# david-jk/BigGAN-Tensorflow

Hardware: AMD Instinct MI355X
Metric: BigGAN-128 train-step images/sec (higher is better)
Workload: dtype bf16; 1 GPU; BigGAN-128 ch=96 bf16 (BASELINE config 3: global batch 256, 32/GPU over 8 GPUs); img_size=128, ch=96, per_gpu_batch=256, global_batch=256, da_policy=full, g_regularization=ortho_cosine, n_labels=0, gan_type=hinge, hip_graph=False, precision=bf16, parallelism=dp1

## Files before the change

biggan-tensorflow_amd/csrc/igemm16.hip:

```cpp
#include <stdlib.h>

#include "common.h"
#include "igemm.h"
#include "igemm16.h"
#include <type_traits>
#include "igemm_dev.h"

namespace bg {

typedef float f32x4_t __attribute__((ext_vector_type(4)));
typedef float f32x16_t __attribute__((ext_vector_type(16)));
typedef __bf16 bf16x8_t __attribute__((ext_vector_type(8)));
typedef short s16x4v __attribute__((ext_vector_type(4)));
typedef short s16x8v __attribute__((ext_vector_type(8)));
typedef __attribute__((address_space(3))) void lds_void_t;
typedef __attribute__((address_space(1))) const void gbl_void_t;
typedef __attribute__((address_space(3))) s16x4v lds_s16x4v;

__device__ uint4 g_zero_page[1024];

__device__ __forceinline__ void glds16(const void* src, unsigned char* lds_wave_base) {
    __builtin_amdgcn_global_load_lds((gbl_void_t*)src, (lds_void_t*)lds_wave_base, 16, 0, 0);
}

// ... 1069 lines not shown
    return 256 * row + 16 * (chunk ^ (((row & 3) << 2) | ((row >> 2) & 3)));
}

template <int MODE>
__global__ __launch_bounds__(256, 2) void tn16_kernel(const TN16Params p) {
    constexpr int BM = 128, BN = 128;
    extern __shared__ __attribute__((aligned(16))) unsigned char smem[];

    const int t = threadIdx.x;
    const int lane = t & 63, w = t >> 6;
    const int wm = w >> 1, wn = w & 1;
    const Gather& g = p.g;

    const int ntile = p.tiles_m * p.tiles_n;
    const int lin = xcd_remap(blockIdx.x, ntile * p.splitk);
    const int zs = lin / ntile;
    const int tile = lin - zs * ntile;
    const int tile_n = tile % p.tiles_n, tile_m = tile / p.tiles_n;
    const int mf0 = tile_m * BM, cb0 = tile_n * BN;
    const int row_begin = zs * p.rows_per_split;
    const int row_end = min(p.M, row_begin + p.rows_per_split);
    const int nsteps = max(0, (row_end - row_begin + TN16_BK - 1) / TN16_BK);

    const int prow = lane >> 4;
    const int ch = (lane & 15) ^ ((prow << 2) | w);
    const int mf = mf0 + 8 * ch;
    int a_kh = 0, a_kw = 0, a_c = mf;
    if (MODE != GATHER_PLAIN) {
        const int tap = mf / p.Ca;
        a_c = mf - tap * p.Ca;
        a_kh = tap / g.k;
        a_kw = tap - a_kh * g.k;
    }
    const bool a_ok = mf < p.Mf;
    const int cb = cb0 + 8 * ch;
    const bool b_ok = cb < p.Cb;
    const __bf16* Ab = reinterpret_cast<const __bf16*>(p.A);
    const __bf16* Bb = reinterpret_cast<const __bf16*>(p.Bv);
    const void* zero = reinterpret_cast<const void*>(g_zero_page);
    int m_next = row_begin + 4 * w + prow;

    auto stage = [&](int buf) {
        unsigned char* sa = smem + buf * (2 * TN16_TILE) + (4 * w) * 256;
        unsigned char* sb = sa + TN16_TILE;
#pragma unroll
        for (int j = 0; j < 4; ++j) {
            const int m = m_next + 16 * j;
            const void* srca = zero;
            const void* srcb = zero;
            if (m < row_end) {
                if (a_ok) {
                    int64_t pix;
                    if (MODE == GATHER_PLAIN) {
                        pix = m;
                    } else {
                        int b, ho, wo;
                        if (p.pow2) {
                            wo = m & (g.Wq - 1);
                            const int r = m >> p.wq_shift;
                            ho = r & (g.Hq - 1);
                            b = r >> p.hq_shift;
                        } else {
                            wo = m % g.Wq;
                            const int r = m / g.Wq;
                            ho = r % g.Hq;
                            b = r / g.Hq;
                        }
                        const int hs = conv_src(ho, a_kh, g.stride, g.pad, g.reflect, g.Hs);
                        const int ws = conv_src(wo, a_kw, g.stride, g.pad, g.reflect, g.Ws);
                        pix = (hs >= 0 && ws >= 0) ? ((int64_t)b * g.Hs + hs) * g.Ws + ws : -1;
                    }
                    if (pix >= 0) srca = Ab + pix * g.ld + a_c;
                }
                if (b_ok) srcb = Bb + (int64_t)m * p.b_ld + cb;
            }
            glds16(srca, sa + j * 16 * 256);
            glds16(srcb, sb + j * 16 * 256);
        }
        m_next += TN16_BK;
    };

    f32x16_t acc[2][2];
#pragma unroll
    for (int i = 0; i < 2; ++i)
#pragma unroll
        for (int j = 0; j < 2; ++j)
#pragma unroll
            for (int r = 0; r < 16; ++r) acc[i][j][r] = 0.f;

    const int kblk = lane >> 5, g16 = (lane >> 4) & 1, q = (lane & 15) >> 2, pq = lane & 3;
    const uint32_t lds0 = static_cast<uint32_t>(
        reinterpret_cast<uintptr_t>((__attribute__((address_space(3))) unsigned char*)smem));
    uint32_t a_ad[2][2], b_ad[2][2];
#pragma unroll
    for (int jj = 0; jj < 2; ++jj) {
        const int row = 8 * kblk + 4 * jj + q;
#pragma unroll
        for (int i = 0; i < 2; ++i) {
            a_ad[i][jj] = lds0 + tr16_swz(row, 4 * (wm * 2 + i) + 2 * g16 + (pq >> 1)) + 8 * (pq & 1);
            b_ad[i][jj] = lds0 + TN16_TILE + tr16_swz(row, 4 * (wn * 2 + i) + 2 * g16 + (pq >> 1)) + 8 * (pq & 1);
        }
    }
    auto operand = [&](uint32_t lo_addr, uint32_t hi_addr) {
        const s16x4v lo = lds_tr16(lo_addr), hi = lds_tr16(hi_addr);
        const s16x8v v = __builtin_shufflevector(lo, hi, 0, 1, 2, 3, 4, 5, 6, 7);
        return __builtin_bit_cast(bf16x8_t, v);
    };

    if (nsteps > 0) stage(0);
    __syncthreads();
    for (int it = 0; it < nsteps; ++it) {
        const int cur = it & 1;
        if (it + 1 < nsteps) stage(cur ^ 1);
        const uint32_t bufoff = (uint32_t)cur * (2u * TN16_TILE);
#pragma unroll
        for (int s = 0; s < TN16_BK / 16; ++s) {
            bf16x8_t a[2], b[2];
#pragma unroll
            for (int i = 0; i < 2; ++i) a[i] = operand(a_ad[i][0] + bufoff + 4096 * s, a_ad[i][1] + bufoff + 4096 * s);
#pragma unroll
            for (int j = 0; j < 2; ++j) b[j] = operand(b_ad[j][0] + bufoff + 4096 * s, b_ad[j][1] + bufoff + 4096 * s);
#pragma unroll
            for (int i = 0; i < 2; ++i)
#pragma unroll
                for (int j = 0; j < 2; ++j)
                    acc[i][j] = __builtin_amdgcn_mfma_f32_32x32x16_bf16(a[i], b[j], acc[i][j], 0, 0, 0);
        }
        __syncthreads();
    }

    float* obase = p.out + (int64_t)zs * p.slab_stride;
#pragma unroll
    for (int i = 0; i < 2; ++i) {
#pragma unroll
        for (int r = 0; r < 16; ++r) {
            const int row = mf0 + wm * 64 + 32 * i + (r & 3) + 8 * (r >> 2) + 4 * (lane >> 5);
            if (row >= p.Mf) continue;
#pragma unroll
            for (int j = 0; j < 2; ++j) {
                const int col = cb0 + wn * 64 + 32 * j + (lane & 31);
                if (col < p.Cb) obase[(int64_t)row * p.out_ld + col] = acc[i][j][r];
            }
        }
    }
}


template <int MODE, int BK, int NBI = 1>
__global__ __launch_bounds__(512, (BK == 32 && NBI == 1) ? 4 : 2) void tn16x_kernel(const TN16Params p) {
    constexpr int TILE = BK * 256;
    constexpr int TNX_STAGE = (2 + NBI) * TILE;
    constexpr int NJ = BK / 16;
    extern __shared__ __attribute__((aligned(16))) unsigned char smem[];

    const int t = threadIdx.x;
    const int lane = t & 63, w = t >> 6;
    const int wm = w >> 1, wn = w & 1;
    const Gather& g = p.g;

    const int ntile = p.tiles_m * p.tiles_n;
    const int lin = xcd_remap(blockIdx.x, ntile * p.splitk);
    const int zs = lin / ntile;
    const int tile = lin - zs * ntile;
    const int tile_n = tile % p.tiles_n, tile_m = tile / p.tiles_n;
    const int mf0 = tile_m * 256, cb0 = tile_n * 128 * NBI;
    const int row_begin = zs * p.rows_per_split;
    const int row_end = min(p.M, row_begin + p.rows_per_split);
    const int nsteps = max(0, (row_end - row_begin + BK - 1) / BK);

    const int prow = lane >> 4;
    const int wq = w & 3, ia = w >> 2;
    const int ch = (lane & 15) ^ ((prow << 2) | wq);
    const int mf = mf0 + 128 * ia + 8 * ch;
    int a_kh = 0, a_kw = 0, a_c = mf;
    if (MODE != GATHER_PLAIN) {
        const int tap = mf / p.Ca;
        a_c = mf - tap * p.Ca;
        a_kh = tap / g.k;
        a_kw = tap - a_kh * g.k;
    }
    const int cb = cb0 + (NBI == 2 ? 128 * ia : 0) + 8 * ch;
    const void* zero = reinterpret_cast<const void*>(g_zero_page);
    int m_next = row_begin + 4 * wq + prow;
    const uint32_t lds0 = static_cast<uint32_t>(
        reinterpret_cast<uintptr_t>((__attribute__((address_space(3))) unsigned char*)smem));

    const int dh = a_kh - g.pad, dw = a_kw - g.pad;
    const unsigned hmax = g.reflect ? 0xffffffffu : (unsigned)g.Hs - 1u;
    const unsigned wmax = g.reflect ? 0xffffffffu : (unsigned)g.Ws - 1u;
    const int h2 = 2 * (g.Hs - 1), w2 = 2 * (g.Ws - 1);
    const int wmask = g.Wq - 1, hmask = g.Hq - 1, bsh = p.wq_shift + p.hq_shift;
    const int a_lim = mf < p.Mf ? row_end : 0, b_lim = cb < p.Cb ? row_end : 0;
    const unsigned char* abase = reinterpret_cast<const unsigned char*>(reinterpret_cast<const __bf16*>(p.A) + a_c);
    const unsigned char* bbase = reinterpret_cast<const unsigned char*>(reinterpret_cast<const __bf16*>(p.Bv) + cb);
    const unsigned ald2 = 2u * (unsigned)g.ld, bld2 = 2u * (unsigned)p.b_ld;

    const uint32_t sa0 = __builtin_amdgcn_readfirstlane(lds0 + ia * TILE + (4 * wq) * 256);
    const uint32_t sb0 = __builtin_amdgcn_readfirstlane(lds0 + (2 + (NBI == 2 ? ia : 0)) * TILE + (4 * wq) * 256);
    auto stage = [&](int slot) {
        const uint32_t sa = sa0 + slot * TNX_STAGE;
        const uint32_t sb = sb0 + slot * TNX_STAGE;
#pragma unroll
        for (int j = 0; j < NJ; ++j) {
            const int m = m_next + 16 * j;
            unsigned pix = (unsigned)m;
            bool ok = m < a_lim;
            if (MODE != GATHER_PLAIN) {
                const int wo = m & wmask, ho = (m >> p.wq_shift) & hmask, b = m >> bsh;
                const int h = __mul24(ho, g.stride) + dh, wsrc = __mul24(wo, g.stride) + dw;
                const int ha = h < 0 ? -h : h, wa = wsrc < 0 ? -wsrc : wsrc;
                const int hr = min(ha, h2 - ha), wr = min(wa, w2 - wa);
                ok = ok & ((unsigned)h <= hmax) & ((unsigned)wsrc <= wmax);
                pix = __umul24(__umul24((unsigned)b, (unsigned)g.Hs) + (unsigned)hr, (unsigned)g.Ws) + (unsigned)wr;
            }
            const void* srca = ok ? static_cast<const void*>(abase + (uint64_t)pix * ald2) : zero;
            glds16_asm(srca, sa + j * 16 * 256);
            if (NBI == 2 || j / (NJ / 2) == ia) {
                const void* srcb = m < b_lim ? static_cast<const void*>(bbase + (uint64_t)(unsigned)m * bld2) : zero;
                glds16_asm(srcb, sb + j * 16 * 256);
            }
        }
        m_next += BK;
    };

    constexpr int NBJ = 2 * NBI;
    f32x16_t acc[2][NBJ];
#pragma unroll
    for (int i = 0; i < 2; ++i)
#pragma unroll
        for (int j = 0; j < NBJ; ++j)
#pragma unroll
            for (int r = 0; r < 16; ++r) acc[i][j][r] = 0.f;

    const int kblk = lane >> 5, g16 = (lane >> 4) & 1, q = (lane & 15) >> 2, pq = lane & 3;
    uint32_t a_ad[2][2], b_ad[NBJ][2];
#pragma unroll
    for (int jj = 0; jj < 2; ++jj) {
        const int row = 8 * kblk + 4 * jj + q;
#pragma unroll
        for (int i = 0; i < 2; ++i)
            a_ad[i][jj] = lds0 + (wm >> 1) * TILE +
                          tr16_swz(row, 4 * ((wm & 1) * 2 + i) + 2 * g16 + (pq >> 1)) + 8 * (pq & 1);
#pragma unroll
        for (int j = 0; j < NBJ; ++j)
            b_ad[j][jj] = lds0 + (2 + (NBI == 2 ? wn : 0)) * TILE +
                          tr16_swz(row, 4 * (NBI == 2 ? j : wn * 2 + j) + 2 * g16 + (pq >> 1)) + 8 * (pq & 1);
    }
    auto operand = [&](uint32_t lo_addr, uint32_t hi_addr) {
        const s16x4v lo = lds_tr16(lo_addr), hi = lds_tr16(hi_addr);
        const s16x8v v = __builtin_shufflevector(lo, hi, 0, 1, 2, 3, 4, 5, 6, 7);
        return __builtin_bit_cast(bf16x8_t, v);
    };

    if (nsteps > 0) stage(0);
    if (nsteps > 1) stage(1);
    auto kstep = [&](int it, auto slot_c) {
        constexpr int SLOT = decltype(slot_c)::value;
        if (it + 1 < nsteps) {
            if (BK == 64 && NBI == 2) asm volatile("s_waitcnt vmcnt(8) lgkmcnt(0)" ::: "memory");
            else if (BK == 64) asm volatile("s_waitcnt vmcnt(6) lgkmcnt(0)" ::: "memory");
            else if (NBI == 2) asm volatile("s_waitcnt vmcnt(4) lgkmcnt(0)" ::: "memory");
            else asm volatile("s_waitcnt vmcnt(3) lgkmcnt(0)" ::: "memory");
        } else
            asm volatile("s_waitcnt vmcnt(0) lgkmcnt(0)" ::: "memory");
        __builtin_amdgcn_s_barrier();
        if (it + 2 < nsteps) stage((SLOT + 2) % 3);
        constexpr uint32_t bufoff = (uint32_t)SLOT * (uint32_t)TNX_STAGE;
#pragma unroll
        for (int s = 0; s < BK / 16; ++s) {
            bf16x8_t a[2], b[NBJ];
#pragma unroll
            for (int i = 0; i < 2; ++i) a[i] = operand(a_ad[i][0] + (bufoff + 4096 * s), a_ad[i][1] + (bufoff + 4096 * s));
#pragma unroll
            for (int j = 0; j < NBJ; ++j) b[j] = operand(b_ad[j][0] + (bufoff + 4096 * s), b_ad[j][1] + (bufoff + 4096 * s));
#pragma unroll
            for (int i = 0; i < 2; ++i)
#pragma unroll
                for (int j = 0; j < NBJ; ++j)
                    acc[i][j] = __builtin_amdgcn_mfma_f32_32x32x16_bf16(a[i], b[j], acc[i][j], 0, 0, 0);
        }
    };
    for (int it = 0; it < nsteps; it += 3) {
        kstep(it, std::integral_constant<int, 0>());
        if (it + 1 < nsteps) kstep(it + 1, std::integral_constant<int, 1>());
        if (it + 2 < nsteps) kstep(it + 2, std::integral_constant<int, 2>());
    }

    float* obase = p.out + (int64_t)zs * p.slab_stride;
#pragma unroll
    for (int i = 0; i < 2; ++i) {
#pragma unroll
        for (int r = 0; r < 16; ++r) {
            const int row = mf0 + wm * 64 + 32 * i + (r & 3) + 8 * (r >> 2) + 4 * (lane >> 5);
            if (row >= p.Mf) continue;
#pragma unroll
            for (int j = 0; j < NBJ; ++j) {
                const int col = cb0 + wn * 32 * NBJ + 32 * j + (lane & 31);
                if (col < p.Cb) obase[(int64_t)row * p.out_ld + col] = acc[i][j][r];
            }
        }
    }
}

template <bool F32>
__global__ __launch_bounds__(256) void reflect_fold_kernel(const void* __restrict__ dxp_, void* __restrict__ dx_, int N,
                                                           int H, int W, int C8, int Hp, int Wp, int pad,
                                                           int accumulate) {
    const int64_t total = (int64_t)N * H * W * C8;
    for (int64_t i = (int64_t)blockIdx.x * 256 + threadIdx.x; i < total; i += (int64_t)gridDim.x * 256) {
        const int c8 = (int)(i % C8);
        int64_t t = i / C8;
        const int w = (int)(t % W);
        t /= W;
        const int h = (int)(t % H);
        const int n = (int)(t / H);
        int hs[3], ws[3], nh = 0, nw = 0;
        hs[nh++] = h + pad;
        if (h >= 1 && pad - h >= 0) hs[nh++] = pad - h;
        if (h <= H - 2 && 2 * (H - 1) - h + pad < Hp && H > 1) hs[nh++] = 2 * (H - 1) - h + pad;
        ws[nw++] = w + pad;
        if (w >= 1 && pad - w >= 0) ws[nw++] = pad - w;
        if (w <= W - 2 && 2 * (W - 1) - w + pad < Wp && W > 1) ws[nw++] = 2 * (W - 1) - w + pad;
        float acc[8];
#pragma unroll
        for (int j = 0; j < 8; ++j) acc[j] = 0.f;
        for (int a = 0; a < nh; ++a)
            for (int b = 0; b < nw; ++b) {
                if (hs[a] >= Hp || ws[b] >= Wp) continue;
                const int64_t off = ((((int64_t)n * Hp + hs[a]) * Wp + ws[b]) * C8 + c8) * 8;
                if (F32) {
                    const float* sp = reinterpret_cast<const float*>(dxp_) + off;
                    const f32x4_t v0 = *reinterpret_cast<const f32x4_t*>(sp), v1 = *reinterpret_cast<const f32x4_t*>(sp + 4);
#pragma unroll
                    for (int j = 0; j < 4; ++j) {
                        acc[j] += v0[j];
                        acc[4 + j] += v1[j];
                    }
                } else {
                    const uint4 r = *reinterpret_cast<const uint4*>(reinterpret_cast<const __bf16*>(dxp_) + off);
                    acc[0] += bf16_lo(r.x); acc[1] += bf16_hi(r.x); acc[2] += bf16_lo(r.y); acc[3] += bf16_hi(r.y);
                    acc[4] += bf16_lo(r.z); acc[5] += bf16_hi(r.z); acc[6] += bf16_lo(r.w); acc[7] += bf16_hi(r.w);
                }
            }
        if (F32) {
            float* o = reinterpret_cast<float*>(dx_) + i * 8;
            f32x4_t v0 = {acc[0], acc[1], acc[2], acc[3]}, v1 = {acc[4], acc[5], acc[6], acc[7]};
            if (accumulate) {
                v0 += *reinterpret_cast<const f32x4_t*>(o);
                v1 += *reinterpret_cast<const f32x4_t*>(o + 4);
            }
            *reinterpret_cast<f32x4_t*>(o) = v0;
            *reinterpret_cast<f32x4_t*>(o + 4) = v1;
        } else {
            __bf16* o = reinterpret_cast<__bf16*>(dx_) + i * 8;
            if (accumulate) {
                const uint4 r = *reinterpret_cast<const uint4*>(o);
                acc[0] += bf16_lo(r.x); acc[1] += bf16_hi(r.x); acc[2] += bf16_lo(r.y); acc[3] += bf16_hi(r.y);
                acc[4] += bf16_lo(r.z); acc[5] += bf16_hi(r.z); acc[6] += bf16_lo(r.w); acc[7] += bf16_hi(r.w);
            }
            uint4 r;
            r.x = pack_bf16x2(acc[0], acc[1]);
            r.y = pack_bf16x2(acc[2], acc[3]);
            r.z = pack_bf16x2(acc[4], acc[5]);
            r.w = pack_bf16x2(acc[6], acc[7]);
            *reinterpret_cast<uint4*>(o) = r;
        }
    }
}

__global__ __launch_bounds__(256) void reflect_fold_scalar_kernel(const float* __restrict__ dxp, float* __restrict__ dx,
                                                                  int N, int H, int W, int C, int Hp, int Wp, int pad,
                                                                  int accumulate) {
    const int64_t total = (int64_t)N * H * W * C;
    for (int64_t i = (int64_t)blockIdx.x * 256 + threadIdx.x; i < total; i += (int64_t)gridDim.x * 256) {
        const int c = (int)(i % C);
        int64_t t = i / C;
        const int w = (int)(t % W);
        t /= W;
        const int h = (int)(t % H);
        const int n = (int)(t / H);
        int hs[3], ws[3], nh = 0, nw = 0;
        hs[nh++] = h + pad;
        if (h >= 1 && pad - h >= 0) hs[nh++] = pad - h;
        if (h <= H - 2 && 2 * (H - 1) - h + pad < Hp) hs[nh++] = 2 * (H - 1) - h + pad;
        ws[nw++] = w + pad;
        if (w >= 1 && pad - w >= 0) ws[nw++] = pad - w;
        if (w <= W - 2 && 2 * (W - 1) - w + pad < Wp) ws[nw++] = 2 * (W - 1) - w + pad;
        float acc = 0.f;
        for (int a = 0; a < nh; ++a)
            for (int b = 0; b < nw; ++b) {
                if (hs[a] >= Hp || ws[b] >= Wp) continue;
                acc += dxp[(((int64_t)n * Hp + hs[a]) * Wp + ws[b]) * C + c];
            }
        dx[i] = accumulate ? dx[i] + acc : acc;
    }
}

int launch_reflect_fold(const void* dxp, void* dx, int f32, int N, int H, int W, int C, int Hp, int Wp, int pad_lo,
                        int accumulate, hipStream_t s) {
    if (C % 8 != 0) {
        BG_REQUIRE(f32, "reflect fold: bf16 tensors need C %% 8 == 0");
        const int64_t n = (int64_t)N * H * W * C;
        int64_t nb = (n + 255) / 256;
        if (nb > 4096) nb = 4096;
        hipLaunchKernelGGL(reflect_fold_scalar_kernel, dim3((unsigned)nb), dim3(256), 0, s, (const float*)dxp, (float*)dx, N,
                           H, W, C, Hp, Wp, pad_lo, accumulate);
        BG_LAUNCH_CHECK();
        return BG_OK;
    }
    const int64_t total = (int64_t)N * H * W * (C / 8);
    int64_t blocks = (total + 255) / 256;
    if (blocks > 4096) blocks = 4096;
    if (f32)
        hipLaunchKernelGGL((reflect_fold_kernel<true>), dim3((unsigned)blocks), dim3(256), 0, s, dxp, dx, N, H, W, C / 8, Hp,
                           Wp, pad_lo, accumulate);
    else
        hipLaunchKernelGGL((reflect_fold_kernel<false>), dim3((unsigned)blocks), dim3(256), 0, s, dxp, dx, N, H, W, C / 8,
                           Hp, Wp, pad_lo, accumulate);
    BG_LAUNCH_CHECK();
    return BG_OK;
}

struct NN16Plan {
    int tn, splitk;
};

static int nn16_steps_min(const NN16Params& p, int mode) {
    int per_axis = p.g.k;
    if (mode == GATHER_TCONV && p.g.pstep > 1) per_axis = max(1, p.g.k / p.g.stride);
    return (per_axis * per_axis * (p.C >> 3) + 7) >> 3;
}

static double nn16_axis_fraction(const Gather& g, int mode, int nq, int n_src) {
    int64_t valid = 0, slots = 0;
    for (int ph = 0; ph < (mode == GATHER_TCONV ? g.pstep : 1); ++ph) {
        int k0 = 0, kstep = 1, nk = g.k;
        if (mode == GATHER_TCONV && g.pstep > 1) {
            kstep = g.stride;
            k0 = (ph + g.pad) % g.stride;
            nk = (g.k - k0 + g.stride - 1) / g.stride;
        }
        for (int q = 0; q < nq; ++q) {
            const int o = q * g.pstep + ph;
            for (int i = 0; i < nk; ++i) {
                const int kk = k0 + i * kstep;
                bool ok;
                if (mode == GATHER_CONV) {
                    const int src = o * g.stride + kk - g.pad;
                    ok = g.reflect || (src >= 0 && src < n_src);
                } else {
                    const int hn = o + g.pad - kk;
                    ok = hn >= 0 && hn % g.stride == 0 && hn / g.stride < n_src;
                }
                valid += ok;
            }
            slots += nk;
        }
    }
    return slots ? (double)valid / (double)slots : 1.0;
}

static double nn16_posmajor_fraction(const NN16Params& p, int mode) {
    const char* e = getenv("BG_NN16_POSMAJOR");
    if (e && atoi(e) == 0) return 1.0;
    const Gather& g = p.g;
    if (g.k <= 1 || g.Nb < 16 || g.Hq <= 0 || g.Wq <= 0 || (int64_t)g.Hq * g.Wq > 40 * 40) return 1.0;
    const double f = nn16_axis_fraction(g, mode, g.Hq, g.Hs) * nn16_axis_fraction(g, mode, g.Wq, g.Ws);
    return f < 0.9 ? f : 1.0;
}

static NN16Plan plan_nn16(const NN16Params& p, int mode, int zdim, bool allow_split) {
    static const int slots = getenv("BG_NN16_SLOTS") ? atoi(getenv("BG_NN16_SLOTS")) : 512;
    const int64_t tm = (p.M + NN16_BM - 1) / NN16_BM;
    int steps = nn16_steps_min(p, mode);
    const double pm = nn16_posmajor_fraction(p, mode);
    if (pm < 1.0) steps = max(1, (int)(steps * pm + 0.5));
    NN16Plan best{4, 1};
    double best_cost = 1e30;
    for (int tn = 4; tn >= 1; --tn) {
        const int bn = 32 * tn;
        const int64_t tiles = tm * ((p.N + bn - 1) / bn) * zdim;
        const double unit = 1.5 + tn;
        const int max_sk = allow_split ? (steps / 4 < 16 ? (steps / 4 < 1 ? 1 : steps / 4) : 16) : 1;
        for (int sk = 1; sk <= max_sk; ++sk) {
            const int64_t rounds = (tiles * sk + slots - 1) / slots;
            double cost = (double)rounds * ((steps + sk - 1) / sk + 2.0) * unit;
            if (sk > 1) cost += 6.0 * unit + 0.02 * sk * (double)tiles / slots * bn;
            if (cost < best_cost - 1e-9) {
                best_cost = cost;
                best = NN16Plan{tn, sk};
            }
        }
    }
    return best;
}

size_t nn16_workspace_bytes(const NN16Params& p, int mode, int zdim, int64_t out_elems) {
    const NN16Plan pl = plan_nn16(p, mode, zdim, true);
    return pl.splitk > 1 ? (size_t)pl.splitk * out_elems * sizeof(float) : 0;
}

static int nn16_mfast(const NN16Params& p, int tiles_m, int tiles_n);

enum { NN16_FORM_TWO = 0, NN16_FORM_RING = 1, NN16_FORM_WIDE = 2, NN16_FORM_PHASED = 3 };
constexpr int NN16X_CUS = 256;
static int nn16_form(const NN16Params& p, int tn, int64_t row_blocks, bool even_phases, bool mirrored, int* xtn) {
    const bool wide_ok = !mirrored && !p.posmajor && p.g.Ws < (1 << 15);
    const bool phased_ok = !mirrored && (!p.posmajor || p.g.Nb % 256 == 0);
    const int64_t wide_blocks = row_blocks * ((p.N + 32 * tn - 1) / (32 * tn));
    const int64_t nb256 = row_blocks * ((p.N + 255) / 256), nb192 = row_blocks * ((p.N + 191) / 192);
    const int64_t last192 = (nb192 + NN16X_CUS - 1) / NN16X_CUS * NN16X_CUS - nb192;
    const int pad192 = (p.N + 191) / 192 * 192, pad_plan = (p.N + 32 * tn - 1) / (32 * tn) * (32 * tn);
    int bn = 0;
    if (phased_ok && p.C >= 384) {
        if (p.N % 256 == 0 && nb256 % NN16X_CUS == 0 && even_phases) bn = 256;
        else if (pad192 <= pad_plan && nb192 >= (even_phases ? 1 : 2) * NN16X_CUS && last192 * 16 <= NN16X_CUS) bn = 192;
    }
    const int rule_bn = bn;
    if (bn == 0) bn = p.N <= 128 ? 128 : (p.N <= 192 ? 192 : 256);
    if (const char* e = getenv("BG_NN16X_BN")) {
        const int v = atoi(e);
        if (v == 128 || v == 192 || v == 256) bn = v;
    }
    *xtn = bn / 32;
    if (const char* e = getenv("BG_NN16_PIPE")) {
        const int v = atoi(e);
        if (v == 3) return phased_ok ? NN16_FORM_PHASED : NN16_FORM_TWO;
        if (v == 2) return wide_ok ? NN16_FORM_WIDE : NN16_FORM_TWO;
        return (v == 1 && p.g.Ws < (1 << 15)) ? NN16_FORM_RING : NN16_FORM_TWO;
    }
    if (rule_bn) return NN16_FORM_PHASED;
    return (wide_ok && p.C <= 192 && tn >= 2 && wide_blocks >= 512) ? NN16_FORM_WIDE : NN16_FORM_TWO;
}

template <int TN, int SLOTS = 2>
static int launch_nn16_ring_inst(const NN16Params& p, dim3 grid, hipStream_t s) {
    constexpr int lds = SLOTS == 3 ? nn16_pipe_lds_bytes(TN, 2, NN16_RING_TAPS) : nn16_lds_bytes(TN, NN16_RING_TAPS);
    if (!lds_opt_in(reinterpret_cast<const void*>(&nn16_kernel<TN, GATHER_TCONV, true, true, SLOTS>), lds)) return BG_ERR_LAUNCH;
    hipLaunchKernelGGL((nn16_kernel<TN, GATHER_TCONV, true, true, SLOTS>), grid, dim3(256), lds, s, p);
    return BG_OK;
}
template <int TN>
static int launch_nn16_ring_tn(const NN16Params& p, int form, dim3 grid, hipStream_t s) {
    return form == NN16_FORM_RING ? launch_nn16_ring_inst<TN, 3>(p, grid, s) : launch_nn16_ring_inst<TN>(p, grid, s);
}

int launch_nn16_ring(NN16Params& p, hipStream_t s) {
    BG_REQUIRE(p.ring == 1 && (p.ring_lines == 1 || p.ring_lines == 2), "nn16 ring launch: ring = 1, ring_lines 1 or 2");
    BG_REQUIRE(p.g.k >= 1 && p.g.k <= NN16_RING_TAPS / 2 && p.g.Ho >= 4 && p.g.Wo >= 4 && p.accumulate == 1,
               "nn16 ring launch: kernel size %d / map %d x %d not supported", p.g.k, p.g.Ho, p.g.Wo);
    BG_REQUIRE(p.C % 8 == 0 && p.N % 8 == 0 && p.g.ld % 8 == 0 && p.out_ld % 8 == 0, "nn16 ring launch: channels %% 8");
    const int npos = p.ring_lines * p.g.Wo + p.ring_lines * (p.g.Ho - p.ring_lines);
    p.g.pstep = 1;
    p.g.Hq = 1;
    p.g.Wq = npos;
    p.M = p.g.Nb * npos;
    p.posmajor = 1;
    p.splitk = 1;
    p.slabs = nullptr;
    p.zfold = 0;
    p.pow2 = 0;
    int tn = 4, best = 1 << 30;
    for (int c = 4; c >= 1; --c) {
        const int padded = (p.N + 32 * c - 1) / (32 * c) * (32 * c);
        if (padded < best) { best = padded; tn = c; }
    }
    p.tiles_m = (p.M + NN16_BM - 1) / NN16_BM;
    p.tiles_n = (p.N + 32 * tn - 1) / (32 * tn);
    p.mfast = nn16_mfast(p, p.tiles_m, p.tiles_n);
    dim3 grid(p.tiles_m * p.tiles_n, 1, 1);
    int xtn;
    const int form = nn16_form(p, tn, 0, true, true, &xtn);
    int rc;
    switch (tn) {
        case 1: rc = launch_nn16_ring_tn<1>(p, form, grid, s); break;
        case 2: rc = launch_nn16_ring_tn<2>(p, form, grid, s); break;
        case 3: rc = launch_nn16_ring_tn<3>(p, form, grid, s); break;
        default: rc = launch_nn16_ring_tn<4>(p, form, grid, s); break;
    }
    if (rc) return rc;
    BG_LAUNCH_CHECK();
    return BG_OK;
}

template <int TN, int MODE, bool PM, int SLOTS = 2, int WM = 2>
static int launch_nn16_inst(const NN16Params& p, dim3 grid, hipStream_t s) {
    constexpr int lds = SLOTS == 3 ? nn16_pipe_lds_bytes(TN, WM) : (WM == 4 ? nn16x_lds_bytes(TN) : nn16_lds_bytes(TN));
    if (!lds_opt_in(reinterpret_cast<const void*>(&nn16_kernel<TN, MODE, PM, false, SLOTS, WM>), lds)) return BG_ERR_LAUNCH;
    if (SLOTS == 2 && WM == 2) prof_kernel("nn16_kernel<%d, %d, %s>", TN, MODE, PM ? "true" : "false");
    else prof_kernel("nn16_kernel<%d, %d, %s, false, %d, %d>", TN, MODE, PM ? "true" : "false", SLOTS, WM);
    hipLaunchKernelGGL((nn16_kernel<TN, MODE, PM, false, SLOTS, WM>), grid, dim3(128 * WM), lds, s, p);
    return BG_OK;
}

template <int TN, int MODE, bool PM>
static int launch_nn16_tn(const NN16Params& p, int form, dim3 grid, hipStream_t s) {
    if (form == NN16_FORM_RING) return launch_nn16_inst<TN, MODE, PM, 3, 2>(p, grid, s);
    if constexpr (!PM)
        if (form == NN16_FORM_WIDE) return launch_nn16_inst<TN, MODE, PM, 3, 4>(p, grid, s);
    return launch_nn16_inst<TN, MODE, PM>(p, grid, s);
}

template <int MODE, bool PM>
static int launch_nn16_pm(const NN16Params& p, int tn, int form, dim3 grid, hipStream_t s) {
    if (form == NN16_FORM_PHASED)
        return tn == 8   ? launch_nn16_inst<8, MODE, PM, 2, 4>(p, grid, s)
               : tn == 6 ? launch_nn16_inst<6, MODE, PM, 2, 4>(p, grid, s)
                         : launch_nn16_inst<4, MODE, PM, 2, 4>(p, grid, s);
    switch (tn) {
        case 1: return launch_nn16_tn<1, MODE, PM>(p, form, grid, s);
        case 2: return launch_nn16_tn<2, MODE, PM>(p, form, grid, s);
        case 3: return launch_nn16_tn<3, MODE, PM>(p, form, grid, s);
        default: return launch_nn16_tn<4, MODE, PM>(p, form, grid, s);
    }
}

template <int MODE>
static int launch_nn16_mode(const NN16Params& p, int tn, int form, dim3 grid, hipStream_t s) {
    return p.posmajor ? launch_nn16_pm<MODE, true>(p, tn, form, grid, s) : launch_nn16_pm<MODE, false>(p, tn, form, grid, s);
}

static int nn16h_taps(const NN16Params& p, int mode, int zdim) {
    const char* e = getenv("BG_NN16_HALO");
    const int use = e ? atoi(e) : 1;
    static const int cmax = getenv("BG_NN16_HALO_CMAX") ? atoi(getenv("BG_NN16_HALO_CMAX")) : 4096;
    const Gather& g = p.g;
    if (!use || p.C > cmax || p.C % 32 || p.N % 8 || g.Hq < NH_T || g.Wq < NH_T || g.Hq % NH_T || g.Wq % NH_T) return 0;
    if (mode == GATHER_CONV) return (g.stride == 1 && g.k == 3 && g.pstep == 1 && zdim == 1) ? 3 : 0;
    if (g.reflect) return 0;
    if (g.stride == 1 && g.k == 3 && g.pstep == 1 && zdim == 1) return 3;
    if (g.stride == 2 && g.k == 4 && g.pstep == 2 && zdim == 4) return 2;
    if (g.stride == 2 && g.k == 3 && g.pad == 1 && g.pstep == 2 && zdim == 4) {
        const char* e3 = getenv("BG_NN16_HALO_K3S2");
        return (e3 && atoi(e3) == 1) ? 2 : 0;
    }
    return 0;
}

template <int NT, int NF, int MODE, int THIN = 0>
static int launch_nn16h_inst(const NN16Params& p, int blocks, hipStream_t s) {
    constexpr int lds = nn16h_lds_bytes<NT, NF>();
    if (!lds_opt_in(reinterpret_cast<const void*>(&nn16h_kernel<NT, NF, MODE, THIN>), lds)) return BG_ERR_LAUNCH;
    if (THIN) prof_kernel("nn16h_kernel<%d, %d, %d, d2s>", NT, NF, MODE);
    else prof_kernel("nn16h_kernel<%d, %d, %d>", NT, NF, MODE);
    hipLaunchKernelGGL((nn16h_kernel<NT, NF, MODE, THIN>), dim3(blocks), dim3(512), lds, s, p);
    return BG_OK;
}

template <int NT, int MODE>
static int launch_nn16h_nf(const NN16Params& p, int nf, int blocks, hipStream_t s) {
    switch (nf) {
        case 1: return launch_nn16h_inst<NT, 1, MODE>(p, blocks, s);
        case 2: return launch_nn16h_inst<NT, 2, MODE>(p, blocks, s);
        case 3: return launch_nn16h_inst<NT, 3, MODE>(p, blocks, s);
        default: return launch_nn16h_inst<NT, 4, MODE>(p, blocks, s);
    }
}

bool nn16h_d2s_ok(const NN16Params& p) {
    const char* e = getenv("BG_THIN_D2S");
    const int use = e ? atoi(e) : 1;
    const Gather& g = p.g;
    return use && p.N == 8 && p.out_ld == 8 && g.k == 3 && g.stride == 2 && g.pad == 1 && !g.reflect && p.C % 32 == 0 &&
           g.Hs % NH_T == 0 && g.Ws % NH_T == 0 && g.Ho == 2 * g.Hs && g.Wo == 2 * g.Ws && !p.bias && !p.stats_part;
}
int launch_nn16h_d2s(const NN16Params& plain, hipStream_t s) {
    BG_REQUIRE(nn16h_d2s_ok(plain), "nn16h depth-to-space form: unsupported geometry");
    NN16Params p = plain;
    Gather& g = p.g;
    g.Hq = g.Hs; g.Wq = g.Ws; g.pstep = 1; g.pad = 0; g.stride = 1;
    p.N = 32;
    p.splitk = 1; p.mfast = 0; p.ring = 0;
    const int64_t blocks = (int64_t)g.Nb * (g.Hq / NH_T) * (g.Wq / NH_T);
    BG_REQUIRE(blocks > 0 && blocks < (int64_t(1) << 31), "nn16h: grid out of range");
    if (const int rc = launch_nn16h_inst<2, 1, GATHER_CONV, 1>(p, (int)blocks, s)) return rc;
    BG_LAUNCH_CHECK();
    return BG_OK;
}

static int nn16_mfast(const NN16Params& p, int tiles_m, int tiles_n) {
    const char* e = getenv("BG_NN16_MFAST");
    if (!e) return 0;
    if (strcmp(e, "auto") != 0) return atoi(e) != 0;
    const double l2 = 3.0e6;
    const double a_bytes = 2.0 * p.g.Nb * (double)p.g.Hs * p.g.Ws * p.g.ld;
    const double w_bytes = 2.0 * p.g.k * p.g.k * (double)p.N * p.C;
    const double nfast = a_bytes + (w_bytes > l2 ? w_bytes * tiles_m : w_bytes);
    const double mfast = w_bytes + (a_bytes > l2 ? a_bytes * tiles_n : a_bytes);
    return mfast < nfast;
}

static int launch_nn16h(NN16Params& p, int mode, int ntaps, hipStream_t s) {
    int nf = 4, best = 1 << 30;
    for (int c = 4; c >= 1; --c) {
        const int padded = (p.N + 32 * c - 1) / (32 * c) * (32 * c);
        if (padded < best) { best = padded; nf = c; }
    }
    const Gather& g = p.g;
    const int64_t blocks = (int64_t)g.Nb * (g.Hq / NH_T) * (g.Wq / NH_T) * ((p.N + 32 * nf - 1) / (32 * nf)) *
                           (g.pstep * g.pstep);
    BG_REQUIRE(blocks > 0 && blocks < (int64_t(1) << 31), "nn16h: grid out of range");
    p.splitk = 1;
    p.mfast = nn16_mfast(p, g.Nb * (g.Hq / NH_T) * (g.Wq / NH_T), (p.N + 32 * nf - 1) / (32 * nf));
    int rc;
    if (mode == GATHER_CONV) rc = launch_nn16h_nf<3, GATHER_CONV>(p, nf, (int)blocks, s);
    else if (ntaps == 3) rc = launch_nn16h_nf<3, GATHER_TCONV>(p, nf, (int)blocks, s);
    else rc = launch_nn16h_nf<2, GATHER_TCONV>(p, nf, (int)blocks, s);
    if (rc) return rc;
    BG_LAUNCH_CHECK();
    return BG_OK;
}

bool nn16_d2s_ok(const NN16Params& p, int mode, int zdim) {
    const Gather& g = p.g;
    if (p.d2s_c <= 0 || p.d2s_c % 8 || p.N != 4 * p.d2s_c || p.C % 8 || mode != GATHER_CONV || zdim != 1 || g.stride != 1 ||
        g.pstep != 1 || g.Hq != g.Ho || g.Wq != g.Wo || p.stats_part || p.ring)
        return false;
    if ((int64_t)g.Nb * g.Ho * g.Wo * 4 >= (int64_t(1) << 31)) return false;
    if (nn16h_taps(p, mode, zdim)) return true;
    if (nn16_posmajor_fraction(p, mode) < 1.0) return false;
    return plan_nn16(p, mode, zdim, true).splitk == 1;
}

int64_t nn16_stats_rows(const NN16Params& p, int mode, int zdim) {
    if (p.C % 8 || p.N % 8 || !nn16h_taps(p, mode, zdim)) return 0;
    return 2 * (int64_t)p.g.Nb * (p.g.Hq / NH_T) * (p.g.Wq / NH_T) * (p.g.pstep * p.g.pstep);
}

int launch_nn16(NN16Params& p, int mode, int zdim, int64_t out_elems, void* ws, size_t ws_bytes, hipStream_t s) {
    BG_REQUIRE(p.C % 8 == 0 && p.N % 8 == 0 && p.g.ld % 8 == 0 && p.out_ld % 8 == 0,
               "bf16-resident conv: channel counts must be multiples of 8 (C=%d N=%d)", p.C, p.N);
    BG_REQUIRE((reinterpret_cast<uintptr_t>(p.A) & 15) == 0 && (reinterpret_cast<uintptr_t>(p.B) & 15) == 0 &&
                   (reinterpret_cast<uintptr_t>(p.out) & 15) == 0,
               "bf16-resident conv: tensors must be 16-byte aligned");
    BG_REQUIRE(p.g.k >= 1 && p.g.k <= NN16_TAPS && p.C <= 8192 && p.g.stride >= 1 && p.g.stride <= 2,
               "bf16-resident conv: kernel size %d / stride %d / %d channels not supported", p.g.k, p.g.stride, p.C);
    BG_REQUIRE((int64_t)p.g.Nb * p.g.Hs * p.g.Ws < (int64_t(1) << 30) && (int64_t)p.g.Nb * p.g.Ho * p.g.Wo < (int64_t(1) << 31),
               "bf16-resident conv: more than 2^30 source / 2^31 output pixels");
    BG_REQUIRE(p.d2s_c == 0 || (nn16_d2s_ok(p, mode, zdim) && ws == nullptr),
               "bf16-resident conv: this launch has no depth-to-space store (bg_conv2d_fwd_d2s_supported)");
    if (const int ntaps = nn16h_taps(p, mode, zdim)) return launch_nn16h(p, mode, ntaps, s);
    BG_REQUIRE(p.stats_part == nullptr, "bf16-resident conv: fused statistics need the halo-tile form (nn16_stats_rows)");
    NN16Plan pl = plan_nn16(p, mode, zdim, ws != nullptr);
    if (pl.splitk > 1 && ws_bytes < (size_t)pl.splitk * out_elems * sizeof(float)) pl.splitk = 1;
    p.splitk = pl.splitk;
    p.slabs = reinterpret_cast<float*>(ws);
    p.slab_stride = out_elems;
    p.posmajor = nn16_posmajor_fraction(p, mode) < 1.0;
    int xtn;
    const int form = nn16_form(p, pl.tn, (int64_t)((p.M + 255) / 256) * zdim * pl.splitk,
                               zdim == 1 || p.g.k % p.g.stride == 0, false, &xtn);
    const int ltn = form == NN16_FORM_PHASED ? xtn : pl.tn;
    const int bn = 32 * ltn;
    p.tiles_n = (p.N + bn - 1) / bn;
    const int bm = (form == NN16_FORM_WIDE || form == NN16_FORM_PHASED) ? 256 : NN16_BM;
    p.tiles_m = (p.M + bm - 1) / bm;
    p.pow2 = 0;
    if (p.g.Wq > 0 && p.g.Hq > 0 && (p.g.Wq & (p.g.Wq - 1)) == 0 && (p.g.Hq & (p.g.Hq - 1)) == 0) {
        p.pow2 = 1;
        p.wq_shift = __builtin_ctz(p.g.Wq);
        p.hq_shift = __builtin_ctz(p.g.Hq);
    }
    p.mfast = nn16_mfast(p, p.tiles_m, p.tiles_n);
    dim3 grid(p.tiles_m * p.tiles_n, 1, zdim * p.splitk);
    p.zfold = 0;
    if (mode == GATHER_TCONV && zdim > 1 && p.splitk == 1 && p.g.k % p.g.stride == 0) {
        p.zfold = zdim;
        grid = dim3(p.tiles_m * p.tiles_n * zdim, 1, 1);
    }
    int rc;
    if (mode == GATHER_CONV)
        rc = launch_nn16_mode<GATHER_CONV>(p, ltn, form, grid, s);
    else
        rc = launch_nn16_mode<GATHER_TCONV>(p, ltn, form, grid, s);
    if (rc) return rc;
    BG_LAUNCH_CHECK();
    if (pl.splitk > 1) {
        const int64_t n8 = out_elems / 8;
        int blocks = (int)((n8 + 255) / 256);
        if (blocks > 2048) blocks = 2048;
        hipLaunchKernelGGL(nn16_slab_reduce_kernel, dim3(blocks), dim3(256), 0, s, p.slabs, p.out, p.bias, p.alpha, n8,
                           p.N, pl.splitk, out_elems, p.accumulate, p.out_f32);
        BG_LAUNCH_CHECK();
    }
    return BG_OK;
}

static void plan_tn16(TN16Params& p) {
    const int64_t tiles = (int64_t)((p.Mf + 127) / 128) * ((p.Cb + 127) / 128);
    static const int want = getenv("BG_TN16_WANT") ? atoi(getenv("BG_TN16_WANT")) : 1024;
    int sk = (int)(want / tiles);
    const int max_sk = (p.M + 4 * TN16_BK - 1) / (4 * TN16_BK);
    if (sk > max_sk) sk = max_sk;
    if (sk < 1) sk = 1;
    if (sk > 512) sk = 512;
    int rps = (p.M + sk - 1) / sk;
    rps = (rps + TN16_BK - 1) / TN16_BK * TN16_BK;
    p.splitk = (p.M + rps - 1) / rps;
    p.rows_per_split = rps;
}

static int tn16x_nbi(const TN16Params& p) {
    const char* e = getenv("BG_TN16X_NBI");
    if (!e || atoi(e) != 2) return 1;
    return (p.Cb >= 512 && p.Cb % 256 == 0 && p.Mf >= 256) ? 2 : 1;
}

static bool plan_tn16x(const TN16Params& p, int* sk_out, int* rps_out) {
    static const int use_wide = getenv("BG_TN16_WIDE") ? atoi(getenv("BG_TN16_WIDE")) : 1;
    if (!use_wide || p.Mf <= 128 || p.M < 8 * TN16_BK) return false;
    if (p.g.k > 0 && (p.g.Wq <= 0 || p.g.Hq <= 0 || (p.g.Wq & (p.g.Wq - 1)) || (p.g.Hq & (p.g.Hq - 1)))) return false;
    const int nbi = tn16x_nbi(p);
    const int tm = (p.Mf + 255) / 256, tn = (p.Cb + 128 * nbi - 1) / (128 * nbi);
    static const int wantx0 = getenv("BG_TN16X_WANT") ? atoi(getenv("BG_TN16X_WANT")) : 512;
    const int wantx = nbi == 2 ? wantx0 / 2 : wantx0;
    int sk = wantx / (tm * tn);
    const int max_sk = (p.M + 4 * TN16_BK - 1) / (4 * TN16_BK);
    if (sk > max_sk) sk = max_sk;
    if (sk < 1) sk = 1;
    if (sk > 512) sk = 512;
    int rps = (p.M + sk - 1) / sk;
    rps = (rps + TN16_BK - 1) / TN16_BK * TN16_BK;
    *sk_out = (p.M + rps - 1) / rps;
    *rps_out = rps;
    return true;
}

size_t tn16_workspace_bytes(const TN16Params& p0) {
    TN16Params p = p0;
    plan_tn16(p);
    int sk = p.splitk, skx = 1, rps = 0;
    if (plan_tn16x(p0, &skx, &rps) && skx > sk) sk = skx;
    return sk > 1 ? (size_t)sk * p.Mf * p.Cb * sizeof(float) : 0;
}

int launch_tn16(TN16Params& p, int mode, float* final_out, void* ws, size_t ws_bytes, hipStream_t s) {
    BG_REQUIRE(p.Ca % 8 == 0 && p.Cb % 8 == 0 && p.g.ld % 8 == 0 && p.b_ld % 8 == 0,
               "bf16-resident wgrad: channel counts must be multiples of 8 (Ca=%d Cb=%d)", p.Ca, p.Cb);
    BG_REQUIRE((reinterpret_cast<uintptr_t>(p.A) & 15) == 0 && (reinterpret_cast<uintptr_t>(p.Bv) & 15) == 0,
               "bf16-resident wgrad: tensors must be 16-byte aligned");
    plan_tn16(p);
    const int64_t total = (int64_t)p.Mf * p.Cb;
    if (p.splitk > 1 && (ws == nullptr || ws_bytes < (size_t)p.splitk * total * sizeof(float) || p.out_ld != p.Cb)) {
        p.splitk = 1;
        p.rows_per_split = (p.M + TN16_BK - 1) / TN16_BK * TN16_BK;
    }
    if (p.splitk > 1) {
        p.out = reinterpret_cast<float*>(ws);
        p.slab_stride = total;
    } else {
        p.out = final_out;
        p.slab_stride = 0;
    }
    p.tiles_m = (p.Mf + 127) / 128;
    p.tiles_n = (p.Cb + 127) / 128;
    p.pow2 = 0;
    if (mode != GATHER_PLAIN && (p.g.Wq & (p.g.Wq - 1)) == 0 && (p.g.Hq & (p.g.Hq - 1)) == 0) {
        p.pow2 = 1;
        p.wq_shift = __builtin_ctz(p.g.Wq);
        p.hq_shift = __builtin_ctz(p.g.Hq);
    }
    int sk = 1, rps = 0;
    if (plan_tn16x(p, &sk, &rps)) {
        const int nbi = tn16x_nbi(p);
        const int tm = (p.Mf + 255) / 256, tn = (p.Cb + 128 * nbi - 1) / (128 * nbi);
        const bool can_split = ws != nullptr && ws_bytes >= (size_t)sk * total * sizeof(float) && p.out_ld == p.Cb;
        if (sk == 1 || can_split) {
            p.splitk = sk;
            p.rows_per_split = rps;
            p.out = sk > 1 ? reinterpret_cast<float*>(ws) : final_out;
            p.slab_stride = sk > 1 ? total : 0;
            p.tiles_m = tm;
            p.tiles_n = tn;
            static const int bk = getenv("BG_TN16X_BK") ? atoi(getenv("BG_TN16X_BK")) : 32;
            if (nbi == 2) {
                constexpr int ldsw = 3 * 4 * 32 * 256;
                const void* fw = mode == GATHER_CONV ? reinterpret_cast<const void*>(&tn16x_kernel<GATHER_CONV, 32, 2>)
                                                     : reinterpret_cast<const void*>(&tn16x_kernel<GATHER_PLAIN, 32, 2>);
                if (!lds_opt_in(fw, ldsw)) return BG_ERR_LAUNCH;
                prof_kernel("tn16x_kernel<%d, 32, 2>", mode == GATHER_CONV ? GATHER_CONV : GATHER_PLAIN);
                dim3 gridw(tm * tn * sk, 1, 1);
                if (mode == GATHER_CONV) hipLaunchKernelGGL((tn16x_kernel<GATHER_CONV, 32, 2>), gridw, dim3(512), ldsw, s, p);
                else hipLaunchKernelGGL((tn16x_kernel<GATHER_PLAIN, 32, 2>), gridw, dim3(512), ldsw, s, p);
                BG_LAUNCH_CHECK();
                if (sk > 1) {
                    launch_slab_reduce(reinterpret_cast<const float*>(ws), final_out, total, sk, total, s);
                    BG_LAUNCH_CHECK();
                }
                return BG_OK;
            }
            const int ldsx = 3 * 3 * bk * 256;
            const void* fx = mode == GATHER_CONV
                                 ? (bk == 64 ? reinterpret_cast<const void*>(&tn16x_kernel<GATHER_CONV, 64>)
                                             : reinterpret_cast<const void*>(&tn16x_kernel<GATHER_CONV, 32>))
                                 : (bk == 64 ? reinterpret_cast<const void*>(&tn16x_kernel<GATHER_PLAIN, 64>)
                                             : reinterpret_cast<const void*>(&tn16x_kernel<GATHER_PLAIN, 32>));
            if (!lds_opt_in(fx, ldsx)) return BG_ERR_LAUNCH;
            prof_kernel("tn16x_kernel<%d, %d>", mode == GATHER_CONV ? GATHER_CONV : GATHER_PLAIN, bk == 64 ? 64 : 32);
            dim3 gridx(tm * tn * sk, 1, 1);
            if (mode == GATHER_CONV) {
                if (bk == 64) hipLaunchKernelGGL((tn16x_kernel<GATHER_CONV, 64>), gridx, dim3(512), ldsx, s, p);
                else hipLaunchKernelGGL((tn16x_kernel<GATHER_CONV, 32>), gridx, dim3(512), ldsx, s, p);
            } else {
                if (bk == 64) hipLaunchKernelGGL((tn16x_kernel<GATHER_PLAIN, 64>), gridx, dim3(512), ldsx, s, p);
                else hipLaunchKernelGGL((tn16x_kernel<GATHER_PLAIN, 32>), gridx, dim3(512), ldsx, s, p);
            }
            BG_LAUNCH_CHECK();
            if (sk > 1) {
                launch_slab_reduce(reinterpret_cast<const float*>(ws), final_out, total, sk, total, s);
                BG_LAUNCH_CHECK();
            }
            return BG_OK;
        }
    }
    dim3 grid(p.tiles_m * p.tiles_n * p.splitk, 1, 1);
    constexpr int lds = 4 * TN16_TILE;
    if (!lds_opt_in(mode == GATHER_CONV ? reinterpret_cast<const void*>(&tn16_kernel<GATHER_CONV>)
                                        : reinterpret_cast<const void*>(&tn16_kernel<GATHER_PLAIN>), lds))
        return BG_ERR_LAUNCH;
    prof_kernel("tn16_kernel<%d>", mode == GATHER_CONV ? GATHER_CONV : GATHER_PLAIN);
    if (mode == GATHER_CONV)
        hipLaunchKernelGGL((tn16_kernel<GATHER_CONV>), grid, dim3(256), lds, s, p);
    else
        hipLaunchKernelGGL((tn16_kernel<GATHER_PLAIN>), grid, dim3(256), lds, s, p);
    BG_LAUNCH_CHECK();
    if (p.splitk > 1) {
        launch_slab_reduce(reinterpret_cast<const float*>(ws), final_out, total, p.splitk, total, s);
        BG_LAUNCH_CHECK();
    }
    return BG_OK;
}

}
```

Baseline: 2818 images/sec.

## Add phased ring-buffered wide TN16 conv weight-grad kernel with wider column tiles

Adds a new tn16x_phased_kernel for the conv-mode TN weight-gradient GEMM. It uses a multi-slot LDS ring (6 or 8 K-blocks), issues async global-to-LDS loads interleaved between the two MFMA halves of each phase, and uses setprio and sched barriers to overlap loads with compute. Column tiles widen to 192 or 256, chosen by a wave-quantization heuristic over 256 CUs. The aim is to hide memory latency and cut tail waste in the wgrad GEMMs, at the cost of more LDS and registers per block and more complex tail handling.

```diff
diff --git a/biggan-tensorflow_amd/csrc/igemm16.hip b/biggan-tensorflow_amd/csrc/igemm16.hip
--- a/biggan-tensorflow_amd/csrc/igemm16.hip
+++ b/biggan-tensorflow_amd/csrc/igemm16.hip
@@ -1395,6 +1395,187 @@
     }
 }
 
+constexpr int tn16xp_lds_bytes(int NKB) { return NKB * 4 * 16 * 256; }
+
+template <int MODE, int BN, int NKB>
+__global__ __launch_bounds__(512, 2) void tn16x_phased_kernel(const TN16Params p) {
+    static_assert(BN == 192 || BN == 256, "column tile: B image 0 and half or all of B image 1");
+    static_assert(NKB >= 3, "ring: the block being read, the block that lands next, at least one more in flight");
+    constexpr int NBJ = BN / 64;
+    constexpr int IMG = 16 * 256;
+    constexpr int KBLK = 4 * IMG;
+    extern __shared__ __attribute__((aligned(16))) unsigned char smem[];
+
+    const int t = threadIdx.x;
+    const int lane = t & 63, w = t >> 6;
+    const int wm = w >> 1, wn = w & 1;
+    const Gather& g = p.g;
+
+    const int ntile = p.tiles_m * p.tiles_n;
+    const int lin = xcd_remap(blockIdx.x, ntile * p.splitk);
+    const int zs = lin / ntile;
+    const int tile = lin - zs * ntile;
+    const int tile_n = tile % p.tiles_n, tile_m = tile / p.tiles_n;
+    const int mf0 = tile_m * 256, cb0 = tile_n * BN;
+    const int row_begin = zs * p.rows_per_split;
+    const int row_end = min(p.M, row_begin + p.rows_per_split);
+    const int nkb = 2 * max(0, (row_end - row_begin + 31) / 32);
+
+    const int prow = lane >> 4;
+    const int wq = w & 3, ia = w >> 2;
+    const int ch = (lane & 15) ^ ((prow << 2) | wq);
+    const int mf = mf0 + 128 * ia + 8 * ch;
+    int a_kh = 0, a_kw = 0, a_c = mf;
+    if (MODE != GATHER_PLAIN) {
+        const int tap = mf / p.Ca;
+        a_c = mf - tap * p.Ca;
+        a_kh = tap / g.k;
+        a_kw = tap - a_kh * g.k;
+    }
+    const int cb = cb0 + 128 * ia + 8 * ch;
+    const bool b_lane = BN == 256 || ia == 0 || ch < 8;
+    const void* zero = reinterpret_cast<const void*>(g_zero_page);
+    int m_next = row_begin + 4 * wq + prow;
+    const uint32_t lds0 = static_cast<uint32_t>(
+        reinterpret_cast<uintptr_t>((__attribute__((address_space(3))) unsigned char*)smem));
+
+    const int dh = a_kh - g.pad, dw = a_kw - g.pad;
+    const unsigned hmax = g.reflect ? 0xffffffffu : (unsigned)g.Hs - 1u;
+    const unsigned wmax = g.reflect ? 0xffffffffu : (unsigned)g.Ws - 1u;
+    const int h2 = 2 * (g.Hs - 1), w2 = 2 * (g.Ws - 1);
+    const int wmask = g.Wq - 1, hmask = g.Hq - 1, bsh = p.wq_shift + p.hq_shift;
+    const int a_lim = mf < p.Mf ? row_end : 0, b_lim = cb < p.Cb ? row_end : 0;
+    const unsigned char* abase = reinterpret_cast<const unsigned char*>(reinterpret_cast<const __bf16*>(p.A) + a_c);
+    const unsigned char* bbase = reinterpret_cast<const unsigned char*>(reinterpret_cast<const __bf16*>(p.Bv) + cb);
+    const unsigned ald2 = 2u * (unsigned)g.ld, bld2 = 2u * (unsigned)p.b_ld;
+
+    const uint32_t sa0 = __builtin_amdgcn_readfirstlane(lds0 + ia * IMG + (4 * wq) * 256);
+    const uint32_t sb0 = __builtin_amdgcn_readfirstlane(lds0 + (2 + ia) * IMG + (4 * wq) * 256);
+    auto issue = [&](int slot) __attribute__((always_inline)) {
+        const int m = m_next;
+        unsigned pix = (unsigned)m;
+        bool ok = m < a_lim;
+        if (MODE != GATHER_PLAIN) {
+            const int wo = m & wmask, ho = (m >> p.wq_shift) & hmask, b = m >> bsh;
+            const int h = __mul24(ho, g.stride) + dh, wsrc = __mul24(wo, g.stride) + dw;
+            const int ha = h < 0 ? -h : h, wa = wsrc < 0 ? -wsrc : wsrc;
+            const int hr = min(ha, h2 - ha), wr = min(wa, w2 - wa);
+            ok = ok & ((unsigned)h <= hmax) & ((unsigned)wsrc <= wmax);
+            pix = __umul24(__umul24((unsigned)b, (unsigned)g.Hs) + (unsigned)hr, (unsigned)g.Ws) + (unsigned)wr;
+        }
+        const void* srca = ok ? static_cast<const void*>(abase + (uint64_t)pix * ald2) : zero;
+        glds16_asm(srca, sa0 + slot * KBLK);
+        const void* srcb = m < b_lim ? static_cast<const void*>(bbase + (uint64_t)(unsigned)m * bld2) : zero;
+        if (b_lane) glds16_asm(srcb, sb0 + slot * KBLK);
+        m_next += 16;
+    };
+
+    f32x16_t acc[2][NBJ];
+#pragma unroll
+    for (int i = 0; i < 2; ++i)
+#pragma unroll
+        for (int j = 0; j < NBJ; ++j)
+#pragma unroll
+            for (int r = 0; r < 16; ++r) acc[i][j][r] = 0.f;
+
+    const int kblk = lane >> 5, g16 = (lane >> 4) & 1, q = (lane & 15) >> 2, pq = lane & 3;
+    uint32_t a_ad[2][2], b_ad[NBJ][2];
+#pragma unroll
+    for (int jj = 0; jj < 2; ++jj) {
+        const int row = 8 * kblk + 4 * jj + q;
+#pragma unroll
+        for (int i = 0; i < 2; ++i)
+            a_ad[i][jj] = lds0 + (wm >> 1) * IMG +
+                          tr16_swz(row, 4 * ((wm & 1) * 2 + i) + 2 * g16 + (pq >> 1)) + 8 * (pq & 1);
+#pragma unroll
+        for (int j = 0; j < NBJ; ++j) {
+            const int f = NBJ * wn + j;
+            b_ad[j][jj] = lds0 + (2 + (f >> 2)) * IMG + tr16_swz(row, 4 * (f & 3) + 2 * g16 + (pq >> 1)) + 8 * (pq & 1);
+        }
+    }
+    auto operand = [&](uint32_t lo_addr, uint32_t hi_addr) __attribute__((always_inline)) {
+        const s16x4v lo = lds_tr16(lo_addr), hi = lds_tr16(hi_addr);
+        const s16x8v v = __builtin_shufflevector(lo, hi, 0, 1, 2, 3, 4, 5, 6, 7);
+        return __builtin_bit_cast(bf16x8_t, v);
+    };
+
+    bf16x8_t ra[2][2], rb[2][NBJ];
+    auto read_block = [&](auto slot_c) __attribute__((always_inline)) {
+        constexpr int SLOT = decltype(slot_c)::value;
+        constexpr uint32_t off = (uint32_t)SLOT * (uint32_t)KBLK;
+#pragma unroll
+        for (int i = 0; i < 2; ++i) ra[SLOT & 1][i] = operand(a_ad[i][0] + off, a_ad[i][1] + off);
+#pragma unroll
+        for (int j = 0; j < NBJ; ++j) rb[SLOT & 1][j] = operand(b_ad[j][0] + off, b_ad[j][1] + off);
+    };
+    auto phase = [&](int n, auto slot_c, auto tail_c) __attribute__((always_inline)) {
+        constexpr int SLOT = decltype(slot_c)::value;
+        constexpr bool TAIL = decltype(tail_c)::value;
+        if (!TAIL || n + NKB <= nkb) asm volatile("s_waitcnt vmcnt(%0) lgkmcnt(0)" ::"n"(2 * (NKB - 2)) : "memory");
+        else asm volatile("s_waitcnt vmcnt(0) lgkmcnt(0)" ::: "memory");
+        __builtin_amdgcn_s_waitcnt(0xC07F);
+        __builtin_amdgcn_s_barrier();
+        __builtin_amdgcn_sched_barrier(0);
+        if (!TAIL || n + 1 < nkb) read_block(std::integral_constant<int, (SLOT + 1) % NKB>());
+        __builtin_amdgcn_s_setprio(1);
+#pragma unroll
+        for (int j = 0; j < NBJ; ++j)
+            acc[0][j] = __builtin_amdgcn_mfma_f32_32x32x16_bf16(ra[SLOT & 1][0], rb[SLOT & 1][j], acc[0][j], 0, 0, 0);
+        __builtin_amdgcn_s_setprio(0);
+        __builtin_amdgcn_sched_barrier(0);
+        if (!TAIL || n + NKB < nkb) issue(SLOT);
+        __builtin_amdgcn_sched_barrier(0);
+        __builtin_amdgcn_s_setprio(1);
+#pragma unroll
+        for (int j = 0; j < NBJ; ++j)
+            acc[1][j] = __builtin_amdgcn_mfma_f32_32x32x16_bf16(ra[SLOT & 1][1], rb[SLOT & 1][j], acc[1][j], 0, 0, 0);
+        __builtin_amdgcn_s_setprio(0);
+        __builtin_amdgcn_sched_barrier(0);
+    };
+    auto round = [&](int n, auto tail_c) __attribute__((always_inline)) {
+        phase(n, std::integral_constant<int, 0>(), tail_c);
+        if (n + 1 < nkb) phase(n + 1, std::integral_constant<int, 1>(), tail_c);
+        if (n + 2 < nkb) phase(n + 2, std::integral_constant<int, 2>(), tail_c);
+        if (n + 3 < nkb) phase(n + 3, std::integral_constant<int, 3>(), tail_c);
+        if (n + 4 < nkb) phase(n + 4, std::integral_constant<int, 4>(), tail_c);
+        if (n + 5 < nkb) phase(n + 5, std::integral_constant<int, 5>(), tail_c);
+        if constexpr (NKB == 8) {
+            if (n + 6 < nkb) phase(n + 6, std::integral_constant<int, 6>(), tail_c);
+            if (n + 7 < nkb) phase(n + 7, std::integral_constant<int, 7>(), tail_c);
+        }
+    };
+    static_assert(NKB == 6 || NKB == 8, "round() spells the phases out");
+
+#pragma unroll
+    for (int k = 0; k < NKB; ++k)
+        if (k < nkb) issue(k);
+    if (nkb >= NKB) asm volatile("s_waitcnt vmcnt(%0)" ::"n"(2 * (NKB - 1)) : "memory");
+    else asm volatile("s_waitcnt vmcnt(0)" ::: "memory");
+    __builtin_amdgcn_s_barrier();
+    if (nkb > 0) read_block(std::integral_constant<int, 0>());
+    const std::integral_constant<bool, false> steady;
+    const std::integral_constant<bool, true> tail;
+    int n = 0;
+    for (; n + 2 * NKB <= nkb; n += NKB) round(n, steady);
+    if (n < nkb) round(n, tail);
+    if (n + NKB < nkb) round(n + NKB, tail);
+
+    float* obase = p.out + (int64_t)zs * p.slab_stride;
+#pragma unroll
+    for (int i = 0; i < 2; ++i) {
+#pragma unroll
+        for (int r = 0; r < 16; ++r) {
+            const int row = mf0 + wm * 64 + 32 * i + (r & 3) + 8 * (r >> 2) + 4 * (lane >> 5);
+            if (row >= p.Mf) continue;
+#pragma unroll
+            for (int j = 0; j < NBJ; ++j) {
+                const int col = cb0 + 32 * (NBJ * wn + j) + (lane & 31);
+                if (col < p.Cb) obase[(int64_t)row * p.out_ld + col] = acc[i][j][r];
+            }
+        }
+    }
+}
+
 template <bool F32>
 __global__ __launch_bounds__(256) void reflect_fold_kernel(const void* __restrict__ dxp_, void* __restrict__ dx_, int N,
                                                            int H, int W, int C8, int Hp, int Wp, int pad,
@@ -1899,6 +2080,36 @@
     return (p.Cb >= 512 && p.Cb % 256 == 0 && p.Mf >= 256) ? 2 : 1;
 }
 
+constexpr int TN16XP_CUS = 256;
+static int tn16x_phased_bn(const TN16Params& p, int mode, int tm, int sk) {
+    if (mode != GATHER_CONV || tn16x_nbi(p) != 1) return 0;
+    int bn = 0;
+    for (int c = 192; c <= 256 && bn == 0; c += 64) {
+        const int64_t blocks = (int64_t)tm * (p.Cb / c) * sk;
+        const int64_t last = (blocks + TN16XP_CUS - 1) / TN16XP_CUS * TN16XP_CUS - blocks;
+        if (p.Cb % c == 0 && last * 2 <= TN16XP_CUS) bn = c;
+    }
+    if (const char* e = getenv("BG_TN16X_PHASED")) {
+        if (atoi(e) == 0) return 0;
+        if (bn == 0) bn = (p.Cb > 192 && p.Cb % 256 == 0) ? 256 : 192;
+    }
+    if (bn == 0) return 0;
+    if (const char* e = getenv("BG_TN16X_PHASED_BN")) {
+        const int v = atoi(e);
+        if (v == 192 || v == 256) bn = v;
+    }
+    return bn;
+}
+
+template <int BN, int NKB>
+static int launch_tn16x_phased(const TN16Params& p, dim3 grid, hipStream_t s) {
+    constexpr int lds = tn16xp_lds_bytes(NKB);
+    if (!lds_opt_in(reinterpret_cast<const void*>(&tn16x_phased_kernel<GATHER_CONV, BN, NKB>), lds)) return BG_ERR_LAUNCH;
+    prof_kernel("tn16x_phased_kernel<%d, %d, %d>", (int)GATHER_CONV, BN, NKB);
+    hipLaunchKernelGGL((tn16x_phased_kernel<GATHER_CONV, BN, NKB>), grid, dim3(512), lds, s, p);
+    return BG_OK;
+}
+
 static bool plan_tn16x(const TN16Params& p, int* sk_out, int* rps_out) {
     static const int use_wide = getenv("BG_TN16_WIDE") ? atoi(getenv("BG_TN16_WIDE")) : 1;
     if (!use_wide || p.Mf <= 128 || p.M < 8 * TN16_BK) return false;
@@ -1966,6 +2177,22 @@
             p.tiles_m = tm;
             p.tiles_n = tn;
             static const int bk = getenv("BG_TN16X_BK") ? atoi(getenv("BG_TN16X_BK")) : 32;
+            if (const int pbn = tn16x_phased_bn(p, mode, tm, sk)) {
+                const char* ring = getenv("BG_TN16X_PHASED_RING");
+                const int nkb = ring ? atoi(ring) : 6;
+                p.tiles_n = (p.Cb + pbn - 1) / pbn;
+                dim3 gridp(tm * p.tiles_n * sk, 1, 1);
+                int rc;
+                if (pbn == 256) rc = nkb == 8 ? launch_tn16x_phased<256, 8>(p, gridp, s) : launch_tn16x_phased<256, 6>(p, gridp, s);
+                else rc = nkb == 8 ? launch_tn16x_phased<192, 8>(p, gridp, s) : launch_tn16x_phased<192, 6>(p, gridp, s);
+                if (rc) return rc;
+                BG_LAUNCH_CHECK();
+                if (sk > 1) {
+                    launch_slab_reduce(reinterpret_cast<const float*>(ws), final_out, total, sk, total, s);
+                    BG_LAUNCH_CHECK();
+                }
+                return BG_OK;
+            }
             if (nbi == 2) {
                 constexpr int ldsw = 3 * 4 * 32 * 256;
                 const void* fw = mode == GATHER_CONV ? reinterpret_cast<const void*>(&tn16x_kernel<GATHER_CONV, 32, 2>)
```

Measured after the change: 2868 images/sec, median of 6. +1.8%, better.
